# 2thleZ/flash_attention_metal

Measured on AMD Instinct MI355X. Metric: attn_fwd_tflops (seqlen=4096, head_dim=64, bf16, causal), higher is better.
Workload: dtype bf16; 1 GPU; BASELINE.json configs[2]: seqlen=4096 head_dim=64 batch=4 heads=16 bf16 is_causal=true per GPU; batch_per_gpu=4, heads=16, seq_len=4096, head_dim=64, is_causal=True

## Files before the change

flash_attention_metal_amd/csrc/fa_mfma16_kernel.hip:

```cpp
#include <stdlib.h>

#include <algorithm>

#include "fa_mfma_common.h"

#ifndef FA16_DEFER_THR
#define FA16_DEFER_THR 8.0f
#endif
#ifndef FA16_LAK
#define FA16_LAK (D == 128 ? 3 : 2)
#endif
#ifndef FA16_LAV
#define FA16_LAV (D == 128 ? 3 : 2)
#endif
#ifndef FA16_PRIO
#define FA16_PRIO 1
#endif
#ifndef FA16_ONES
#define FA16_ONES 1
#endif
#ifndef FA16_LAZY
#define FA16_LAZY 1
#endif
#ifndef FA16_LAZY_THR
#define FA16_LAZY_THR 0x1p20f
#endif
#ifndef FA16_LAZY_POISON
#define FA16_LAZY_POISON 0x1p64f
#endif
#ifndef FA16_HALVES
#define FA16_HALVES 0
#endif
#ifndef FA16_BN128
#define FA16_BN128 64
#endif
#ifndef FA16_OCC128
#define FA16_OCC128 2
#endif
#ifndef FA16_SUB8
#define FA16_SUB8 1
#endif
#ifndef FA16_OCC
#define FA16_OCC 4
#endif

namespace fa {

typedef float f32x4 __attribute__((ext_vector_type(4)));

template <typename Tag> struct MT16;
template <> struct MT16<BF16> {
  using elem = __bf16;
  using vec8 = bf16x8;
  __device__ static __forceinline__ f32x4 mfma(vec8 a, vec8 b, f32x4 c) { return __builtin_amdgcn_mfma_f32_16x16x32_bf16(a, b, c, 0, 0, 0); }
};
template <> struct MT16<F16> {
  using elem = _Float16;
  using vec8 = f16x8;
  __device__ static __forceinline__ f32x4 mfma(vec8 a, vec8 b, f32x4 c) { return __builtin_amdgcn_mfma_f32_16x16x32_f16(a, b, c, 0, 0, 0); }
};

__device__ __forceinline__ float xlane(float x, int mask) { return __shfl_xor(x, mask, 64); }

template <typename Tag, int D, int SUB>
constexpr size_t mfma16_lds_bytes() {
  constexpr bool lazy = std::is_same<Tag, BF16>::value && D == 64 && (FA16_ONES != 0) && (FA16_LAZY == 1);
  return 4 * SUB * (size_t)(D == 128 ? FA16_BN128 : BN) * D * 2 + (lazy ? 16 : 0);
}

template <typename Tag, int D, bool CAUSAL, int RW, bool PAD, int SUB>
__device__ __forceinline__ void fwd_mfma16_body(const Params &p) {
  using M = MT16<Tag>;
  using vec8 = typename M::vec8;
  using elem = typename M::elem;
  constexpr int BMR = RW * WM;
  constexpr int RB = D * 2;
  constexpr int CPR = D / 8;
  constexpr int KS = D / 32;
  constexpr int DT = D / 16;
  constexpr int BNK = (D == 128) ? FA16_BN128 : BN;
  constexpr int KT = BNK / 16;
  constexpr int NKP = KT / 2;
  constexpr int TILE = BNK * RB;
  static_assert(D == 64 || D == 128, "head dims of the 16x16x32 kernel");

  extern __shared__ __attribute__((aligned(16))) char smem_generic[];
  lds_char *smem = (lds_char *)smem_generic;
  lds_char *Kbuf = smem;
  lds_char *Vbuf = smem + 2 * SUB * TILE;

  const int wave = __builtin_amdgcn_readfirstlane((int)threadIdx.x >> 6);
  const int lane = threadIdx.x & 63;
  const int c = lane & 15;
  const int g = lane >> 4;

  int bh, qb;
  map_block<CAUSAL>(blockIdx.x, p, bh, qb);
  long long base, base_kv;
  head_bases(bh, p, base, base_kv);
  const int coff = p.Nk - p.N;
  const int q0 = qb * BMR;
  const int qw0 = q0 + wave * WM;

  const int GRB = PAD ? p.D * 2 : RB;
  auto gcol = [&](int chunk) -> unsigned { return (!PAD || chunk * 8 < p.D) ? (unsigned)chunk * 16 : 0x80000000u; };
  const unsigned head_bytes = (unsigned)p.N * GRB, kv_head_bytes = (unsigned)p.Nk * GRB;
  const __amdgpu_buffer_rsrc_t rq = __builtin_amdgcn_make_buffer_rsrc((void *)((const char *)p.q + base * 2), 0, head_bytes, 0x00020000);
  const __amdgpu_buffer_rsrc_t rk = __builtin_amdgcn_make_buffer_rsrc((void *)((const char *)p.k + base_kv * 2), 0, kv_head_bytes, 0x00020000);
  const __amdgpu_buffer_rsrc_t rv = __builtin_amdgcn_make_buffer_rsrc((void *)((const char *)p.v + base_kv * 2), 0, kv_head_bytes, 0x00020000);

  vec8 qf[2][KS];
#pragma unroll
  for (int qt = 0; qt < 2; ++qt)
#pragma unroll
    for (int ks = 0; ks < KS; ++ks) {
      const u32x4 t = __builtin_amdgcn_raw_buffer_load_b128(rq, (unsigned)(qw0 + 16 * qt + c) * GRB + gcol(4 * ks + g), 0, 0);
      qf[qt][ks] = __builtin_bit_cast(vec8, t);
    }

  const int kx = (D == 64) ? ((c >> 1) & 7) : c;
  const lds_char *kptr[KS];
#pragma unroll
  for (int ks = 0; ks < KS; ++ks) {
    kptr[ks] = Kbuf + c * RB + (((4 * ks + g) ^ kx) << 4);
    asm volatile("" : "+v"(kptr[ks]));
  }
  const int vq = c >> 2, vp = c & 3;
  const int vrow = 4 * g + vq;
  const int vx = (D == 64) ? (((vrow >> 1) & 3) << 1) : ((vrow & 7) << 1);
  const lds_char *vptr[DT];
#pragma unroll
  for (int dt = 0; dt < DT; ++dt) {
    vptr[dt] = Vbuf + vrow * RB + ((((2 * dt) ^ vx) + (vp >> 1)) << 4) + 8 * (vp & 1);
    asm volatile("" : "+v"(vptr[dt]));
  }

  const int kv_end = CAUSAL ? min(p.Nk, q0 + BMR + coff) : p.Nk;
  const int nT = (kv_end + BNK - 1) / BNK;

  constexpr int RPP = 1024 / RB;
  constexpr int NPW = (BNK / RPP) / RW;
  static_assert((RW * RPP) % 16 == 0, "the piece stride must keep the swizzle");
  unsigned dma_kvo, dma_vvo;
  {
    const int row = wave * RPP + lane / CPR, pc = lane % CPR;
    const int skx = (D == 64) ? ((row >> 1) & 7) : (row & 15);
    const int svx = (D == 64) ? (((row >> 1) & 3) << 1) : ((row & 7) << 1);
    dma_kvo = (unsigned)(row * GRB) + gcol(pc ^ skx);
    dma_vvo = (unsigned)(row * GRB) + gcol(pc ^ svx);
  }
  auto stage_dma = [&](int t, int buf) {
#pragma unroll
    for (int j = 0; j < NPW; ++j) {
      const unsigned soff = PAD ? (unsigned)(t * BNK + j * RW * RPP) * GRB : (unsigned)t * TILE + j * (RW * 1024);
      const unsigned lk = (unsigned)(__UINTPTR_TYPE__)Kbuf + buf * TILE + (wave + RW * j) * 1024;
      const unsigned lv = (unsigned)(__UINTPTR_TYPE__)Vbuf + buf * TILE + (wave + RW * j) * 1024;
      asm volatile("s_mov_b32 m0, %0\n\ts_nop 0\n\tbuffer_load_dwordx4 %1, %2, %3 offen lds" ::"s"(lk), "v"(dma_kvo), "s"(rk), "s"(soff) : "memory");
      asm volatile("s_mov_b32 m0, %0\n\ts_nop 0\n\tbuffer_load_dwordx4 %1, %2, %3 offen lds" ::"s"(lv), "v"(dma_vvo), "s"(rv), "s"(soff) : "memory");
    }
  };

  f32x4 oacc[DT][2];
#pragma unroll
  for (int dt = 0; dt < DT; ++dt)
#pragma unroll
    for (int qt = 0; qt < 2; ++qt)
#pragma unroll
      for (int i = 0; i < 4; ++i) oacc[dt][qt][i] = 0.0f;
  constexpr bool ONES = (FA16_ONES != 0);
  constexpr bool LAZY = ONES && std::is_same<Tag, BF16>::value && D == 64 && (FA16_LAZY != 0);
  constexpr bool LAZY_TEST = LAZY && (FA16_LAZY == 1);
  static_assert(4 * SUB * TILE + (LAZY_TEST ? 4 : 0) <= mfma16_lds_bytes<Tag, D, SUB>() && RW * WM * RB <= 4 * SUB * TILE,
                "the launcher's LDS size covers the K / V buffers, the flag word and the epilogue's O tiles");
  lds_char *poison_flag = smem + 4 * SUB * TILE;
  int slow = 0;
  constexpr float BIAS = !ONES ? 0.0f : std::is_same<Tag, F16>::value ? 3.0f : 7.0f;
  constexpr float FIRST_SUM_FLOOR = std::is_same<Tag, F16>::value ? 1.0f : 0x1p-64f;
  float l[2] = {0.0f, 0.0f};
  f32x4 lacc[2];
#pragma unroll
  for (int qt = 0; qt < 2; ++qt)
#pragma unroll
    for (int i = 0; i < 4; ++i) lacc[qt][i] = 0.0f;
  vec8 ones;
#pragma unroll
  for (int j = 0; j < 8; ++j) ones[j] = (elem)1.0f;
  if constexpr (ONES) asm volatile("" : "+v"(ones));
  const float c2 = p.scale * 1.4426950408889634f;
  f32x4 negm[2];
#pragma unroll
  for (int qt = 0; qt < 2; ++qt) {
#pragma unroll
    for (int i = 0; i < 4; ++i) negm[qt][i] = ONES ? -BIAS : INFINITY;
    asm volatile("" : "+v"(negm[qt]));
  }

  if constexpr (LAZY_TEST) {
    if (threadIdx.x == 0) lds_write_b32(poison_flag, 0u);
  }
  stage_dma(0, 0);
  if constexpr (SUB == 2) {
    if (1 < nT) stage_dma(1, 1);
  }
  asm volatile("s_waitcnt vmcnt(0)" ::: "memory");
#pragma unroll
  for (int qt = 0; qt < 2; ++qt)
#pragma unroll
    for (int ks = 0; ks < KS; ++ks) {
#pragma unroll
      for (int j = 0; j < 8; ++j) qf[qt][ks][j] = (elem)((float)qf[qt][ks][j] * c2);
      asm volatile("" : "+v"(qf[qt][ks]));
    }
  __syncthreads();

  const float sum_thr = __builtin_exp2f(FA16_DEFER_THR);
  auto apply_mask = [&](auto k0c, auto &s, const int kv0) __attribute__((always_inline)) {
    constexpr int K0 = decltype(k0c)::value;
    constexpr int NKT = sizeof(s) / sizeof(s[0]);
    int g4 = 4 * g;
    asm volatile("" : "+v"(g4));
#pragma unroll
    for (int qt = 0; qt < 2; ++qt) {
      int lim = p.Nk - 1 - kv0 - g4;
      if (CAUSAL) lim = min(lim, qw0 + 16 * qt + c + coff - kv0 - g4);
#pragma unroll
      for (int k2 = 0; k2 < NKT; ++k2)
#pragma unroll
        for (int i = 0; i < 4; ++i) s[k2][qt][i] = (16 * (K0 + k2) + i > lim) ? -INFINITY : s[k2][qt][i];
    }
  };
  auto needs_mask = [&](const int kv0) __attribute__((always_inline)) { return (CAUSAL && (kv0 + BNK - 1 > qw0 + coff)) || (kv0 + BNK > p.Nk); };
  auto score_group = [&](auto bufc, auto k0c, auto &s, const f32x4 c0, const f32x4 c1) __attribute__((always_inline)) {
    constexpr int buf = decltype(bufc)::value;
    constexpr int K0 = decltype(k0c)::value;
    constexpr int NKT = sizeof(s) / sizeof(s[0]);
    constexpr int NK = NKT * KS, LA = (FA16_LAK < NK) ? FA16_LAK : NK;
    vec8 kf[NK];
    auto kread = [&](int i) { kf[i] = __builtin_bit_cast(vec8, lds_read_b128(kptr[i % KS] + buf * TILE + (K0 + i / KS) * 16 * RB)); };
#pragma unroll
    for (int i = 0; i < LA; ++i) kread(i);
    __builtin_amdgcn_sched_barrier(0);
#pragma unroll
    for (int i = 0; i < NK; ++i) {
      const int k2 = i / KS, ks = i % KS;
      s[k2][0] = M::mfma(kf[i], qf[0][ks], ks == 0 ? c0 : s[k2][0]);
      s[k2][1] = M::mfma(kf[i], qf[1][ks], ks == 0 ? c1 : s[k2][1]);
      if (i + LA < NK) kread(i + LA);
      __builtin_amdgcn_sched_barrier(0);
    }
  };
  auto pack_group = [&](auto k0c, auto &s, vec8 (&pf)[NKP][2], unsigned &bits) __attribute__((always_inline)) {
    constexpr int K0 = decltype(k0c)::value;
    constexpr int NKT = sizeof(s) / sizeof(s[0]);
#pragma unroll
    for (int kp = 0; kp < NKT / 2; ++kp)
#pragma unroll
      for (int qt = 0; qt < 2; ++qt) {
#pragma unroll
        for (int j = 0; j < 8; ++j) pf[K0 / 2 + kp][qt][j] = (elem)s[2 * kp + (j >> 2)][qt][j & 3];
        if constexpr (ONES && !LAZY) {
          const u32x4 w = __builtin_bit_cast(u32x4, pf[K0 / 2 + kp][qt]);
          bits |= w[0] | w[1] | w[2] | w[3];
        }
      }
  };
  auto hot_group = [&](auto bufc, auto k0c, auto nktc, const int kv0, vec8 (&pf)[NKP][2], unsigned &bits, float (&ls)[2],
                       const bool leave) __attribute__((always_inline)) -> bool {
    constexpr int NKT = decltype(nktc)::value;
    f32x4 s[NKT][2];
    score_group(bufc, k0c, s, negm[0], negm[1]);
    if constexpr (LAZY_TEST) {
      if (__builtin_expect(leave, 0)) return true;
    }
    if (needs_mask(kv0)) apply_mask(k0c, s, kv0);
#if FA16_PRIO
    if constexpr (decltype(k0c)::value + NKT == KT) __builtin_amdgcn_s_setprio(0);
#endif
#pragma unroll
    for (int k2 = 0; k2 < NKT; ++k2)
#pragma unroll
      for (int i = 0; i < 4; ++i)
#pragma unroll
        for (int qt = 0; qt < 2; ++qt) {
          s[k2][qt][i] = __builtin_amdgcn_exp2f(s[k2][qt][i]);
          if constexpr (!ONES) ls[qt] = (decltype(k0c)::value == 0 && k2 == 0 && i == 0) ? s[k2][qt][i] : ls[qt] + s[k2][qt][i];
        }
    pack_group(k0c, s, pf, bits);
    return false;
  };
  auto max_group = [&](auto bufc, auto k0c, auto nktc, const int kv0, float (&mx)[2]) __attribute__((always_inline)) {
    constexpr int NKT = decltype(nktc)::value;
    f32x4 s[NKT][2], zero;
#pragma unroll
    for (int i = 0; i < 4; ++i) zero[i] = 0.0f;
    score_group(bufc, k0c, s, zero, zero);
    if (needs_mask(kv0)) apply_mask(k0c, s, kv0);
#pragma unroll
    for (int qt = 0; qt < 2; ++qt)
#pragma unroll
      for (int k2 = 0; k2 < NKT; ++k2)
#pragma unroll
        for (int i = 0; i < 4; ++i) mx[qt] = fmaxf(mx[qt], s[k2][qt][i]);
  };
  auto new_reference = [&](auto firstc, float (&mx)[2]) __attribute__((always_inline)) {
    constexpr bool FIRST = decltype(firstc)::value;
#pragma unroll
    for (int qt = 0; qt < 2; ++qt) {
      float v = mx[qt];
      v = fmaxf(v, xlane(v, 16));
      v = fmaxf(v, xlane(v, 32));
      const float m_old = -negm[qt][0];
      const float m_new = FIRST ? v + BIAS : fmaxf(m_old, v + BIAS);
#pragma unroll
      for (int i = 0; i < 4; ++i) negm[qt][i] = -m_new;
      asm volatile("" : "+v"(negm[qt]));
      if constexpr (FIRST) continue;
      const float alpha = __builtin_amdgcn_exp2f(m_old - m_new);
      if constexpr (ONES) {
#pragma unroll
        for (int i = 0; i < 4; ++i) lacc[qt][i] *= alpha;
      } else {
        l[qt] *= alpha;
      }
#pragma unroll
      for (int dt = 0; dt < DT; ++dt)
#pragma unroll
        for (int i = 0; i < 4; ++i) oacc[dt][qt][i] *= alpha;
    }
  };
  constexpr unsigned LAZY_THR_BITS = __builtin_bit_cast(unsigned, (float)FA16_LAZY_THR);
  constexpr unsigned LAZY_POISON_BITS = __builtin_bit_cast(unsigned, (float)FA16_LAZY_POISON);
  static_assert(LAZY_THR_BITS < LAZY_POISON_BITS && LAZY_POISON_BITS < 0x7f800000u, "2^-BIAS << THR < POISON < inf");
  auto lazy_renormalise = [&]() __attribute__((always_inline)) {
    const unsigned b0 = __builtin_bit_cast(unsigned, lacc[0][0]), b1 = __builtin_bit_cast(unsigned, lacc[1][0]);
    if (__builtin_expect(__builtin_amdgcn_ballot_w64(max(b0, b1) >= LAZY_THR_BITS) != 0, 0)) {
#pragma unroll
      for (int qt = 0; qt < 2; ++qt) {
        const unsigned a = __builtin_bit_cast(unsigned, lacc[qt][0]) & 0x7fffffffu;
        const bool bad = a >= LAZY_POISON_BITS;
        const bool big = !bad && a >= LAZY_THR_BITS;
        const int e = (int)(a >> 23) - 127;
        const float sc = big ? __builtin_bit_cast(float, (unsigned)(127 - e) << 23) : 1.0f;
        const float kf = big ? (float)e : 0.0f;
#pragma unroll
        for (int i = 0; i < 4; ++i) {
          lacc[qt][i] *= sc;
          negm[qt][i] -= kf;
        }
        asm volatile("" : "+v"(negm[qt]));
#pragma unroll
        for (int dt = 0; dt < DT; ++dt)
#pragma unroll
          for (int i = 0; i < 4; ++i) oacc[dt][qt][i] *= sc;
        if (bad) lds_write_b32(poison_flag, 1u);
      }
    }
  };
  constexpr int G = (FA16_HALVES != 0) ? 2 : 1;
  using KTG = std::integral_constant<int, KT / G>;
  using K0A = std::integral_constant<int, 0>;
  using K0B = std::integral_constant<int, KT / 2>;

  auto tile = [&](auto bufc, auto firstc, const int t) {
    constexpr int buf = decltype(bufc)::value;
    constexpr bool FIRST = decltype(firstc)::value;
    const int kv0 = t * BNK;

    int always = 1;
    if constexpr (!CAUSAL) asm volatile("" : "+s"(always));
    const bool wave_active = CAUSAL ? (kv0 <= qw0 + WM - 1 + coff) : (always != 0);
    if (wave_active) {
      vec8 pf[NKP][2];
      float ls[2] = {0.0f, 0.0f};
      if constexpr (LAZY_TEST && !FIRST) lazy_renormalise();
      bool redo = FIRST && !ONES;
      for (;;) {
        if (__builtin_expect(redo, 0)) {
          float mx[2] = {-INFINITY, -INFINITY};
          max_group(bufc, K0A{}, std::integral_constant<int, KT / 2>{}, kv0, mx);
          max_group(bufc, K0B{}, std::integral_constant<int, KT / 2>{}, kv0, mx);
          new_reference(firstc, mx);
        }
#if FA16_PRIO
        __builtin_amdgcn_s_setprio(1);
#endif
        unsigned bits = 0;
        if constexpr (LAZY_TEST) {
          if (hot_group(bufc, K0A{}, KTG{}, kv0, pf, bits, ls, slow != 0 && !redo)) {
            redo = true;
            continue;
          }
        } else {
          hot_group(bufc, K0A{}, KTG{}, kv0, pf, bits, ls, false);
        }
        if constexpr (G == 2) hot_group(bufc, K0B{}, KTG{}, kv0, pf, bits, ls, false);
        bool stale;
        if constexpr (LAZY) stale = false;
        else if constexpr (ONES) stale = __builtin_amdgcn_ballot_w64((bits & 0x40004000u) != 0) != 0;
        else stale = __builtin_amdgcn_ballot_w64(fmaxf(ls[0], ls[1]) > sum_thr) != 0;
        if (__builtin_expect(stale && !redo, 0)) {
          redo = true;
          continue;
        }
        if constexpr (!ONES) {
          l[0] += ls[0];
          l[1] += ls[1];
        }
#if FA16_PRIO
        __builtin_amdgcn_s_setprio(1);
#endif
        {
          constexpr int NV = NKP * DT, LA = FA16_LAV;
          s16x4 wlo[NV], whi[NV];
          auto vread = [&](int j) {
            const lds_char *vb = vptr[j % DT] + buf * TILE + (32 * (j / DT)) * RB;
            wlo[j] = lds_read_tr16(vb);
            whi[j] = lds_read_tr16(vb + 16 * RB);
          };
#pragma unroll
          for (int j = 0; j < LA; ++j) vread(j);
          __builtin_amdgcn_sched_barrier(0);
#pragma unroll
          for (int j = 0; j < NV; ++j) {
            const s16x8 v8 = __builtin_shufflevector(wlo[j], whi[j], 0, 1, 2, 3, 4, 5, 6, 7);
#pragma unroll
            for (int qt = 0; qt < 2; ++qt) oacc[j % DT][qt] = M::mfma(__builtin_bit_cast(vec8, v8), pf[j / DT][qt], oacc[j % DT][qt]);
            if (j + LA < NV) vread(j + LA);
            if constexpr (ONES) {
              if (j % DT == DT - 1) {
#pragma unroll
                for (int qt = 0; qt < 2; ++qt) lacc[qt] = M::mfma(ones, pf[j / DT][qt], lacc[qt]);
              }
            }
            __builtin_amdgcn_sched_barrier(0);
          }
        }
#if FA16_PRIO
        __builtin_amdgcn_s_setprio(0);
#endif
        if constexpr (FIRST && ONES) {
          if (__builtin_expect(!redo && __builtin_amdgcn_ballot_w64(fminf(lacc[0][0], lacc[1][0]) < FIRST_SUM_FLOOR) != 0, 0)) {
#pragma unroll
            for (int qt = 0; qt < 2; ++qt) {
#pragma unroll
              for (int i = 0; i < 4; ++i) lacc[qt][i] = 0.0f;
#pragma unroll
              for (int dt = 0; dt < DT; ++dt)
#pragma unroll
                for (int i = 0; i < 4; ++i) oacc[dt][qt][i] = 0.0f;
            }
            redo = true;
            continue;
          }
        }
        break;
      }
    }
  };
  auto unit = [&](auto bufc, auto firstc, const int t0) {
    constexpr int buf = decltype(bufc)::value;
#pragma unroll
    for (int sub = 0; sub < SUB; ++sub)
      if (t0 + SUB + sub < nT) stage_dma(t0 + SUB + sub, (buf ^ 1) * SUB + sub);
    tile(std::integral_constant<int, buf * SUB>{}, firstc, t0);
    if constexpr (SUB == 2) {
      if (t0 + 1 < nT) tile(std::integral_constant<int, buf * SUB + 1>{}, std::false_type{}, t0 + 1);
    }
    if (t0 + SUB < nT) asm volatile("s_waitcnt vmcnt(0)" ::: "memory");
    if constexpr (LAZY_TEST) {
      if (t0 + SUB >= nT && slow == 0) {
        const unsigned a0 = __builtin_bit_cast(unsigned, lacc[0][0]) & 0x7fffffffu, a1 = __builtin_bit_cast(unsigned, lacc[1][0]) & 0x7fffffffu;
        if (max(a0, a1) >= LAZY_POISON_BITS) lds_write_b32(poison_flag, 1u);
      }
    }
    __syncthreads();
  };
  for (;;) {
    unit(std::integral_constant<int, 0>{}, std::true_type{}, 0);
    for (int t = SUB; t < nT; t += 2 * SUB) {
      unit(std::integral_constant<int, 1>{}, std::false_type{}, t);
      if (t + SUB < nT) unit(std::integral_constant<int, 0>{}, std::false_type{}, t + SUB);
    }
    if constexpr (LAZY_TEST) {
      if (slow == 0) {
        const unsigned f = *reinterpret_cast<const volatile __attribute__((address_space(3))) unsigned *>(poison_flag);
        if (__builtin_expect(__builtin_amdgcn_readfirstlane((int)f) != 0, 0)) {
          slow = 1;
#pragma unroll
          for (int qt = 0; qt < 2; ++qt) {
#pragma unroll
            for (int i = 0; i < 4; ++i) {
              lacc[qt][i] = 0.0f;
              negm[qt][i] = -BIAS;
            }
            asm volatile("" : "+v"(negm[qt]));
#pragma unroll
            for (int dt = 0; dt < DT; ++dt)
#pragma unroll
              for (int i = 0; i < 4; ++i) oacc[dt][qt][i] = 0.0f;
          }
          stage_dma(0, 0);
          if constexpr (SUB == 2) {
            if (1 < nT) stage_dma(1, 1);
          }
          asm volatile("s_waitcnt vmcnt(0)" ::: "memory");
          __syncthreads();
          continue;
        }
      }
    }
    break;
  }

  int elane = lane;
  if constexpr (LAZY_TEST) asm volatile("" : "+v"(elane));
  const int ec = elane & 15, eg = elane >> 4;
  lds_char *Ot = smem + wave * (WM * RB);
#pragma unroll
  for (int qt = 0; qt < 2; ++qt) {
    float lt = ONES ? lacc[qt][0] : l[qt];
    if constexpr (!ONES) {
      lt += xlane(lt, 16);
      lt += xlane(lt, 32);
    }
    const float inv_l = __builtin_amdgcn_rcpf(lt);
    const int row = 16 * qt + ec, qrow = qw0 + row;
    if (p.lse != nullptr && eg == 0 && qrow < p.N)
      p.lse[(long long)bh * p.N + qrow] = (__builtin_amdgcn_logf(lt) - negm[qt][0]) * 0.6931471805599453f;
#pragma unroll
    for (int dt = 0; dt < DT; ++dt) {
      typedef elem elem4 __attribute__((ext_vector_type(4)));
      elem4 e;
#pragma unroll
      for (int i = 0; i < 4; ++i) e[i] = (elem)(oacc[dt][qt][i] * inv_l);
      const u32x2 w = __builtin_bit_cast(u32x2, e);
      const int ch = (2 * dt + (eg >> 1)) ^ (row & (CPR - 1));
      lds_write_b64(Ot + row * RB + (ch << 4) + 8 * (eg & 1), w);
    }
  }
  __syncthreads();
  {
    elem *Og = (elem *)p.o + base;
#pragma unroll
    for (int it = 0; it < WM * CPR / 64; ++it) {
      const int idx = it * 64 + elane;
      const int row = idx / CPR, ch = idx % CPR;
      const u32x4 vv = lds_read_b128(Ot + row * RB + ((ch ^ (row & (CPR - 1))) << 4));
      if (qw0 + row < p.N && (!PAD || ch * 8 < p.D)) *reinterpret_cast<u32x4 *>(Og + (long long)(qw0 + row) * (PAD ? p.D : D) + ch * 8) = vv;
    }
  }
}

template <typename Tag, int D, bool CAUSAL, int RW, bool PAD = false, int SUB = 1>
__global__ __launch_bounds__(64 * RW, (D == 64 ? FA16_OCC : FA16_OCC128)) void fwd_mfma16_kernel(Params p) {
  fwd_mfma16_body<Tag, D, CAUSAL, RW, PAD, SUB>(p);
}

bool mfma16_supported(int dtype, int D) { return (dtype == FA_DTYPE_F16 || dtype == FA_DTYPE_BF16) && D >= 8 && D <= 128 && D % 8 == 0; }

template <typename Tag, int D, bool CAUSAL, int RW, bool PAD = false, int SUB = 1>
static hipError_t launch16_one(const Params &p, hipStream_t s) {
  int head_group = causal_head_group(p, D, 2);
#ifdef FA16_FORCE_HEAD_GROUP
  head_group = FA16_FORCE_HEAD_GROUP;
#endif
  return launch_blocks(fwd_mfma16_kernel<Tag, D, CAUSAL, RW, PAD, SUB>, p, RW * WM, 64 * RW, mfma16_lds_bytes<Tag, D, SUB>(), head_group, s);
}

int mfma16_waves(int D, int BH, int N, int Nk, int is_causal) {
#ifdef FA16_FORCE_RW
  return FA16_FORCE_RW;
#endif
  if (D != 64 && D != 128) return 4;
  const long long b256 = (long long)BH * ((N + 255) / 256);
  if (D == 128) return (!is_causal && Nk >= 8192 && b256 >= 1024) ? 8 : 4;
  if (!is_causal) return (Nk >= 512 && b256 >= 512) ? 8 : 4;
  return (Nk >= 4096 && Nk < 6144 && b256 >= 1024 && b256 < 1280) ? 8 : 4;
}

hipError_t launch_mfma16(const Params &p, int dtype, hipStream_t s) {
  const bool w8 = mfma16_waves(p.D, p.B * p.H, p.N, p.Nk, p.is_causal) == 8 && (p.D == 64 || !p.is_causal);
  return with_tag(dtype, [&](auto tag) -> hipError_t {
    using Tag = decltype(tag);
    if (p.D != 64 && p.D != 128) {
      if (p.D < 64) return p.is_causal ? launch16_one<Tag, 64, true, 4, true>(p, s) : launch16_one<Tag, 64, false, 4, true>(p, s);
      return p.is_causal ? launch16_one<Tag, 128, true, 4, true>(p, s) : launch16_one<Tag, 128, false, 4, true>(p, s);
    }
    if (p.D == 64) {
      if (w8) return p.is_causal ? launch16_one<Tag, 64, true, 8, false, FA16_SUB8>(p, s) : launch16_one<Tag, 64, false, 8, false, FA16_SUB8>(p, s);
      return p.is_causal ? launch16_one<Tag, 64, true, 4>(p, s) : launch16_one<Tag, 64, false, 4>(p, s);
    }
    if (p.D == 128) {
      if (w8) return launch16_one<Tag, 128, false, 8>(p, s);
      return p.is_causal ? launch16_one<Tag, 128, true, 4>(p, s) : launch16_one<Tag, 128, false, 4>(p, s);
    }
    return hipErrorInvalidValue;
  });
}

}
```

Before: 1127 TFLOP/s.

## Overlap lazy renormalise check with PV MFMAs and precompute causal mask predicate

The lazy-renormalisation ballot test moves from the front of each tile into the PV MFMA loop, so its latency hides behind matrix work, and the rare repair runs after PV. The per-tile mask decision becomes a single scalar sign test computed once per tile and shared by the max and hot score groups. The slow path now redoes the max pass whenever the slow flag is set. The end-of-sequence poison test is taken out of the per-unit tail and run once after the loop, removing a branch from the last unit. The trade-off is more control-flow variants and a renormalisation that now happens one step later, after PV has already accumulated.

```diff
diff --git a/flash_attention_metal_amd/csrc/fa_mfma16_kernel.hip b/flash_attention_metal_amd/csrc/fa_mfma16_kernel.hip
--- a/flash_attention_metal_amd/csrc/fa_mfma16_kernel.hip
+++ b/flash_attention_metal_amd/csrc/fa_mfma16_kernel.hip
@@ -27,6 +27,15 @@
 #endif
 #ifndef FA16_LAZY_POISON
 #define FA16_LAZY_POISON 0x1p64f
+#endif
+#ifndef FA16_LOOK
+#define FA16_LOOK 1
+#endif
+#ifndef FA16_COLD
+#define FA16_COLD 3
+#endif
+#ifndef FA16_TAIL
+#define FA16_TAIL 1
 #endif
 #ifndef FA16_HALVES
 #define FA16_HALVES 0
@@ -170,6 +179,9 @@
   constexpr bool ONES = (FA16_ONES != 0);
   constexpr bool LAZY = ONES && std::is_same<Tag, BF16>::value && D == 64 && (FA16_LAZY != 0);
   constexpr bool LAZY_TEST = LAZY && (FA16_LAZY == 1);
+  constexpr bool LOOK_PV = LAZY_TEST && (FA16_LOOK == 1), LOOK_FRONT = LAZY_TEST && (FA16_LOOK == 0);
+  constexpr bool COLD3 = LAZY_TEST && (FA16_COLD == 3);
+  constexpr bool TAIL_OUT = LAZY_TEST && (FA16_TAIL == 1);
   static_assert(4 * SUB * TILE + (LAZY_TEST ? 4 : 0) <= mfma16_lds_bytes<Tag, D, SUB>() && RW * WM * RB <= 4 * SUB * TILE,
                 "the launcher's LDS size covers the K / V buffers, the flag word and the epilogue's O tiles");
   lds_char *poison_flag = smem + 4 * SUB * TILE;
@@ -265,14 +277,18 @@
       }
   };
   auto hot_group = [&](auto bufc, auto k0c, auto nktc, const int kv0, vec8 (&pf)[NKP][2], unsigned &bits, float (&ls)[2],
-                       const bool leave) __attribute__((always_inline)) -> bool {
+                       const bool leave, const int masked) __attribute__((always_inline)) -> bool {
     constexpr int NKT = decltype(nktc)::value;
     f32x4 s[NKT][2];
     score_group(bufc, k0c, s, negm[0], negm[1]);
-    if constexpr (LAZY_TEST) {
-      if (__builtin_expect(leave, 0)) return true;
-    }
-    if (needs_mask(kv0)) apply_mask(k0c, s, kv0);
+    if constexpr (COLD3) {
+      if (masked < 0) apply_mask(k0c, s, kv0);
+    } else {
+      if constexpr (LAZY_TEST && FA16_COLD != 2) {
+        if (__builtin_expect(leave, 0)) return true;
+      }
+      if (needs_mask(kv0)) apply_mask(k0c, s, kv0);
+    }
 #if FA16_PRIO
     if constexpr (decltype(k0c)::value + NKT == KT) __builtin_amdgcn_s_setprio(0);
 #endif
@@ -288,13 +304,13 @@
     pack_group(k0c, s, pf, bits);
     return false;
   };
-  auto max_group = [&](auto bufc, auto k0c, auto nktc, const int kv0, float (&mx)[2]) __attribute__((always_inline)) {
+  auto max_group = [&](auto bufc, auto k0c, auto nktc, const int kv0, float (&mx)[2], const int masked) __attribute__((always_inline)) {
     constexpr int NKT = decltype(nktc)::value;
     f32x4 s[NKT][2], zero;
 #pragma unroll
     for (int i = 0; i < 4; ++i) zero[i] = 0.0f;
     score_group(bufc, k0c, s, zero, zero);
-    if (needs_mask(kv0)) apply_mask(k0c, s, kv0);
+    if (COLD3 ? masked < 0 : needs_mask(kv0)) apply_mask(k0c, s, kv0);
 #pragma unroll
     for (int qt = 0; qt < 2; ++qt)
 #pragma unroll
@@ -331,29 +347,30 @@
   constexpr unsigned LAZY_THR_BITS = __builtin_bit_cast(unsigned, (float)FA16_LAZY_THR);
   constexpr unsigned LAZY_POISON_BITS = __builtin_bit_cast(unsigned, (float)FA16_LAZY_POISON);
   static_assert(LAZY_THR_BITS < LAZY_POISON_BITS && LAZY_POISON_BITS < 0x7f800000u, "2^-BIAS << THR < POISON < inf");
-  auto lazy_renormalise = [&]() __attribute__((always_inline)) {
+  auto lazy_look = [&]() __attribute__((always_inline)) -> unsigned long long {
     const unsigned b0 = __builtin_bit_cast(unsigned, lacc[0][0]), b1 = __builtin_bit_cast(unsigned, lacc[1][0]);
-    if (__builtin_expect(__builtin_amdgcn_ballot_w64(max(b0, b1) >= LAZY_THR_BITS) != 0, 0)) {
-#pragma unroll
-      for (int qt = 0; qt < 2; ++qt) {
-        const unsigned a = __builtin_bit_cast(unsigned, lacc[qt][0]) & 0x7fffffffu;
-        const bool bad = a >= LAZY_POISON_BITS;
-        const bool big = !bad && a >= LAZY_THR_BITS;
-        const int e = (int)(a >> 23) - 127;
-        const float sc = big ? __builtin_bit_cast(float, (unsigned)(127 - e) << 23) : 1.0f;
-        const float kf = big ? (float)e : 0.0f;
-#pragma unroll
-        for (int i = 0; i < 4; ++i) {
-          lacc[qt][i] *= sc;
-          negm[qt][i] -= kf;
-        }
-        asm volatile("" : "+v"(negm[qt]));
-#pragma unroll
-        for (int dt = 0; dt < DT; ++dt)
-#pragma unroll
-          for (int i = 0; i < 4; ++i) oacc[dt][qt][i] *= sc;
-        if (bad) lds_write_b32(poison_flag, 1u);
-      }
+    return __builtin_amdgcn_ballot_w64(max(b0, b1) >= LAZY_THR_BITS);
+  };
+  auto lazy_repair = [&]() __attribute__((always_inline)) {
+#pragma unroll
+    for (int qt = 0; qt < 2; ++qt) {
+      const unsigned a = __builtin_bit_cast(unsigned, lacc[qt][0]) & 0x7fffffffu;
+      const bool bad = a >= LAZY_POISON_BITS;
+      const bool big = !bad && a >= LAZY_THR_BITS;
+      const int e = (int)(a >> 23) - 127;
+      const float sc = big ? __builtin_bit_cast(float, (unsigned)(127 - e) << 23) : 1.0f;
+      const float kf = big ? (float)e : 0.0f;
+#pragma unroll
+      for (int i = 0; i < 4; ++i) {
+        lacc[qt][i] *= sc;
+        negm[qt][i] -= kf;
+      }
+      asm volatile("" : "+v"(negm[qt]));
+#pragma unroll
+      for (int dt = 0; dt < DT; ++dt)
+#pragma unroll
+        for (int i = 0; i < 4; ++i) oacc[dt][qt][i] *= sc;
+      if (bad) lds_write_b32(poison_flag, 1u);
     }
   };
   constexpr int G = (FA16_HALVES != 0) ? 2 : 1;
@@ -372,13 +389,22 @@
     if (wave_active) {
       vec8 pf[NKP][2];
       float ls[2] = {0.0f, 0.0f};
-      if constexpr (LAZY_TEST && !FIRST) lazy_renormalise();
-      bool redo = FIRST && !ONES;
+      if constexpr (LOOK_FRONT && !FIRST) {
+        if (__builtin_expect(lazy_look() != 0, 0)) lazy_repair();
+      }
+      int masked = 0;
+      if constexpr (COLD3) {
+        const int to_diagonal = CAUSAL ? (qw0 + coff) - (kv0 + BNK - 1) : 0, to_end = p.Nk - (kv0 + BNK);
+        masked = to_diagonal | to_end;
+        asm volatile("" : "+s"(masked));
+      }
+      unsigned long long look = 0;
+      bool redo = (FIRST && !ONES) || (COLD3 && slow != 0);
       for (;;) {
         if (__builtin_expect(redo, 0)) {
           float mx[2] = {-INFINITY, -INFINITY};
-          max_group(bufc, K0A{}, std::integral_constant<int, KT / 2>{}, kv0, mx);
-          max_group(bufc, K0B{}, std::integral_constant<int, KT / 2>{}, kv0, mx);
+          max_group(bufc, K0A{}, std::integral_constant<int, KT / 2>{}, kv0, mx, masked);
+          max_group(bufc, K0B{}, std::integral_constant<int, KT / 2>{}, kv0, mx, masked);
           new_reference(firstc, mx);
         }
 #if FA16_PRIO
@@ -386,14 +412,14 @@
 #endif
         unsigned bits = 0;
         if constexpr (LAZY_TEST) {
-          if (hot_group(bufc, K0A{}, KTG{}, kv0, pf, bits, ls, slow != 0 && !redo)) {
+          if (hot_group(bufc, K0A{}, KTG{}, kv0, pf, bits, ls, !COLD3 && slow != 0 && !redo, masked)) {
             redo = true;
             continue;
           }
         } else {
-          hot_group(bufc, K0A{}, KTG{}, kv0, pf, bits, ls, false);
-        }
-        if constexpr (G == 2) hot_group(bufc, K0B{}, KTG{}, kv0, pf, bits, ls, false);
+          hot_group(bufc, K0A{}, KTG{}, kv0, pf, bits, ls, false, 0);
+        }
+        if constexpr (G == 2) hot_group(bufc, K0B{}, KTG{}, kv0, pf, bits, ls, false, 0);
         bool stale;
         if constexpr (LAZY) stale = false;
         else if constexpr (ONES) stale = __builtin_amdgcn_ballot_w64((bits & 0x40004000u) != 0) != 0;
@@ -432,12 +458,21 @@
                 for (int qt = 0; qt < 2; ++qt) lacc[qt] = M::mfma(ones, pf[j / DT][qt], lacc[qt]);
               }
             }
+            if constexpr (LOOK_PV && !FIRST) {
+              if (j == 0) {
+                look = lazy_look();
+                asm volatile("" : "+s"(look));
+              }
+            }
             __builtin_amdgcn_sched_barrier(0);
           }
         }
 #if FA16_PRIO
         __builtin_amdgcn_s_setprio(0);
 #endif
+        if constexpr (LOOK_PV && !FIRST) {
+          if (__builtin_expect(look != 0, 0)) lazy_repair();
+        }
         if constexpr (FIRST && ONES) {
           if (__builtin_expect(!redo && __builtin_amdgcn_ballot_w64(fminf(lacc[0][0], lacc[1][0]) < FIRST_SUM_FLOOR) != 0, 0)) {
 #pragma unroll
@@ -457,6 +492,10 @@
       }
     }
   };
+  auto tail_test = [&]() __attribute__((always_inline)) {
+    const unsigned a0 = __builtin_bit_cast(unsigned, lacc[0][0]) & 0x7fffffffu, a1 = __builtin_bit_cast(unsigned, lacc[1][0]) & 0x7fffffffu;
+    if (max(a0, a1) >= LAZY_POISON_BITS) lds_write_b32(poison_flag, 1u);
+  };
   auto unit = [&](auto bufc, auto firstc, const int t0) {
     constexpr int buf = decltype(bufc)::value;
 #pragma unroll
@@ -466,20 +505,28 @@
     if constexpr (SUB == 2) {
       if (t0 + 1 < nT) tile(std::integral_constant<int, buf * SUB + 1>{}, std::false_type{}, t0 + 1);
     }
-    if (t0 + SUB < nT) asm volatile("s_waitcnt vmcnt(0)" ::: "memory");
-    if constexpr (LAZY_TEST) {
-      if (t0 + SUB >= nT && slow == 0) {
-        const unsigned a0 = __builtin_bit_cast(unsigned, lacc[0][0]) & 0x7fffffffu, a1 = __builtin_bit_cast(unsigned, lacc[1][0]) & 0x7fffffffu;
-        if (max(a0, a1) >= LAZY_POISON_BITS) lds_write_b32(poison_flag, 1u);
-      }
-    }
-    __syncthreads();
+    if constexpr (TAIL_OUT) {
+      if (t0 + SUB < nT) {
+        asm volatile("s_waitcnt vmcnt(0)" ::: "memory");
+        __syncthreads();
+      }
+    } else {
+      if (t0 + SUB < nT) asm volatile("s_waitcnt vmcnt(0)" ::: "memory");
+      if constexpr (LAZY_TEST) {
+        if (t0 + SUB >= nT && slow == 0) tail_test();
+      }
+      __syncthreads();
+    }
   };
   for (;;) {
     unit(std::integral_constant<int, 0>{}, std::true_type{}, 0);
     for (int t = SUB; t < nT; t += 2 * SUB) {
       unit(std::integral_constant<int, 1>{}, std::false_type{}, t);
       if (t + SUB < nT) unit(std::integral_constant<int, 0>{}, std::false_type{}, t + SUB);
+    }
+    if constexpr (TAIL_OUT) {
+      if (slow == 0) tail_test();
+      __syncthreads();
     }
     if constexpr (LAZY_TEST) {
       if (slow == 0) {
```

After: 1149 TFLOP/s (median of 6 runs). +1.9%, better.
